# cgisky1980/Qwen3-TTS-Rust

Measured on AMD Instinct MI355X. Metric: audio_sec_per_s, higher is better.
Workload: dtype bf16

## Files before the change

include/q3tts.h:

```cpp
#ifndef Q3TTS_H
#define Q3TTS_H

#include <stdint.h>

#ifdef __cplusplus
extern "C" {
#endif

#define Q3TTS_OK 0
#define Q3TTS_ERR_INVALID (-1)
#define Q3TTS_ERR_DEVICE (-2)
#define Q3TTS_ERR_OOM (-3)
#define Q3TTS_ERR_IO (-4)
#define Q3TTS_ERR_STATE (-5)
#define Q3TTS_ERR_UNSUPPORTED (-6)
#define Q3TTS_MAX_BATCH 256

#define Q3TTS_MAX_UPSAMPLE 4
#define Q3TTS_MAX_DEC_BLOCKS 8


typedef struct q3tts_model_config {
    int32_t t_n_layer, t_d_model, t_n_head, t_n_kv_head, t_head_dim, t_d_ffn, t_vocab;
    float t_rope_theta;
// ... 334 lines not shown
int q3tts_k_bgemm_voc(int32_t device, const uint16_t* xb, int32_t B, int32_t K, const uint16_t* w_bf16, int32_t N, int32_t epilogue, const float* bias,
                      int32_t bias_n, const float* col_scale, int32_t seg_rows, int32_t gap_rows, float* y, uint16_t* yb, int32_t want_yb);
int q3tts_k_project(int32_t device, const float* x, int32_t rows, int32_t n_in, const float* w, const float* bias, int32_t n_out, const float* nw,
                    float* y, uint16_t* xb, float* ssp);
int q3tts_k_norm_inputs(int32_t device, const float* x, int32_t rows, int32_t d, const float* nw, uint16_t* xb, float* ssp);
int q3tts_k_alloc_upload(q3tts_engine* e, int64_t bytes, int64_t* mismatches);
int q3tts_k_pcm_pack(int32_t device, const float* src, int32_t rows, int64_t stride, const int32_t* ent_row, const int32_t* ent_first,
                     const int32_t* ent_count, const int64_t* ent_dst, int32_t n_ent, int32_t format, void* out, int64_t out_n);
int q3tts_k_resample_table(int32_t rate_in, int32_t rate_out, int32_t* L, int32_t* M, int32_t* H, float* tab, int64_t cap, int64_t* n);
int q3tts_k_pcm_resample(int32_t device, const float* src, int32_t rows, int64_t stride, const int32_t* row_len, const int32_t* row_final,
                         const int32_t* ent_row, const int32_t* ent_first, const int32_t* ent_count, const int64_t* ent_dst, int32_t n_ent,
                         int32_t rate_in, int32_t rate_out, int32_t format, void* out, int64_t out_n, int32_t iters, float* mean_ms);
int q3tts_k_row_buckets(int32_t max_batch, int32_t* out, int32_t cap);
int q3tts_k_bucket_steps(const q3tts_engine* e, int64_t* out, int32_t cap);
int q3tts_k_prefix_stats(const q3tts_engine* e, int64_t* out2);
int q3tts_k_engine_footprint(const q3tts_engine_config* cfg, int64_t* bytes);
int q3tts_k_device_bytes(const q3tts_engine* e, int64_t* bytes);
int q3tts_k_rng_f32(uint64_t seed, int32_t n, float* out);

#ifdef __cplusplus
}
#endif
#endif
```

qwen3-tts-rust_amd/csrc/q3_admit.hip:

```cpp
#include "q3_engine.h"

#include <chrono>
#include <cstring>

int q3_request_rules(const q3tts_request* r, bool keep, int keep_rows, const char** msg) {
    *msg = !r ? "null request"
         : keep && r->prefix ? "keep-voice: a request that names a prefix cannot keep one"
         : keep && (keep_rows < 0 || (keep_rows == 0 && (r->prompt_embd || !r->prompt))) ? "keep-voice: voice_rows >= 1 with prompt_embd (a prompt_embd request states its voice rows), >= 0 with a prompt built from ids"
         : (r->text_open == 1) && !(r->text_stream == 1) ? "text_open needs text_stream = 1"
         : (r->text_stream == 1) && (r->prompt_embd || !r->prompt || r->prompt->n_text < 1 || !r->prompt->text_ids) ? "text_stream needs a prompt built from ids (prompt), not prompt_embd, with n_text >= 1 (its first text id is the prompt's last row)"
         : "";
    return **msg ? Q3TTS_ERR_INVALID : Q3TTS_OK;
}
int q3_voice_job_rules(const q3tts_prompt_desc* p, const float* embd, int n_tok, const char** msg) {
    *msg = (p != nullptr) == (embd != nullptr) ? "give exactly one of a voice desc or host rows" : embd && n_tok < 1 ? "host rows come with n_tok >= 1" : "";
    return **msg ? Q3TTS_ERR_INVALID : Q3TTS_OK;
}
static int voice_job_check(q3tts_engine* e, const q3tts_prompt_desc* p, const float* embd, int n_tok) {
    const char* msg = "";
    if (q3_voice_job_rules(p, embd, n_tok, &msg) != Q3TTS_OK) return q3_set_err(e, Q3TTS_ERR_INVALID, std::string("prefix: ") + msg);
    if (embd && n_tok >= e->cfg.n_ctx) return q3_set_err(e, Q3TTS_ERR_INVALID, "prefix: n_tok outside 1 .. n_ctx - 1");
    return Q3TTS_OK;
}

// ... 91 lines not shown
static void copy_prefixes(q3tts_engine* e, const std::vector<Adm>& grp, Q3KvPrefix& kp) {
    int n_launch = 0; long long n_prefixed = 0;
    for (const Adm& a : grp) if (a.P > 0) { kvp_add(kp, false, a.r->prefix, a.r->prefix->P, a.b, e->stream, &n_launch); ++n_prefixed; }
    e->kvp_launches.fetch_add(n_launch + (kp.n > 0 ? 1 : 0), std::memory_order_relaxed);
    if (n_prefixed > e->kvp_group_max.load(std::memory_order_relaxed)) e->kvp_group_max.store(n_prefixed, std::memory_order_relaxed);
}
static int save_keeps(q3tts_engine* e, const std::vector<Adm>& grp, const Q3KvPrefix& kp) {
    Q3KvPrefix sv = kp; sv.n = 0;
    int bad = 0, n_launch = 0;
    for (const Adm& a : grp) if (a.keep && !bad) bad = kvp_add(sv, true, a.keep, a.keep_rows, a.b, e->stream, &n_launch);
    if (sv.n == 0) return Q3TTS_OK;
    if (bad || kvp_launch(sv, true, e->stream)) return q3_set_err(e, Q3TTS_ERR_INVALID, "prefix save: launch refused for this model shape");
    Q3_HIP(e, hipGetLastError());
    return Q3TTS_OK;
}
static int seed_slot(q3tts_engine* e, const Adm& a) {
    const q3tts_model_config& m = e->cfg.model;
    hipStream_t s = e->stream;
    const q3tts_request* r = a.r;
    const int b = a.b;
    Q3Lane& L = e->lane;
    const int row = e->row_of_slot[b];
    q3_launch_copy_rows(L.T.x + (size_t)row * m.t_d_model, m.t_d_model, e->pf.x + (size_t)(a.row0 + a.n - 1) * m.t_d_model, m.t_d_model, 1, m.t_d_model, s);
    if (q3_launch_gemm(e, e->T, q3_gemm_head(e->T, 0, m.t_vocab, e->pf, a.row0 + a.n - 1, 1, m.rms_eps, 0, L.logits + (size_t)row * m.t_vocab), s))
        return q3_set_err(e, Q3TTS_ERR_INVALID, "prefill head: launch refused for this model shape");
    float temperature = e->temperature, top_p = e->top_p; int top_k = e->top_k, has_seed = e->has_seed; uint64_t seed = e->seed;
    if (!r->use_engine_sampler) { temperature = r->temperature; top_k = r->top_k; top_p = r->top_p; has_seed = r->has_seed; seed = r->seed; }
    if (!has_seed) seed = wall_seed();
    if (temperature > 0.0f) {
        std::vector<float> draws(a.max_steps);
        q3_stdrng_f32(seed, a.max_steps, draws.data());
        Q3_HIP(e, hipMemcpyAsync(e->rng + (size_t)b * e->cfg.max_steps_cap, draws.data(), (size_t)a.max_steps * 4, hipMemcpyHostToDevice, s));
        Q3_HIP(e, hipStreamSynchronize(s));
    }
    if (e->p_temperature > 0.0f) {
        const size_t per = (size_t)(m.n_codebooks - 1), nd = (size_t)a.max_steps * per;
        std::vector<float> draws(nd);
        q3_stdrng_f32(seed ^ 0x9E3779B97F4A7C15ull, (int)nd, draws.data());
        Q3_HIP(e, hipMemcpyAsync(e->prng + (size_t)b * e->cfg.max_steps_cap * per, draws.data(), nd * 4, hipMemcpyHostToDevice, s));
        Q3_HIP(e, hipStreamSynchronize(s));
    }
    if (e->rep_penalty != 1.0f) Q3_HIP(e, hipMemsetAsync(e->seen + (size_t)b * e->seen_words, 0, (size_t)e->seen_words * 4, s));
    Q3Slot* st = e->slots_host + e->B + b;
    memset(st, 0, sizeof(*st));
    st->active = 1; st->cur_pos = a.P + a.n; st->n_frames = 0; st->max_steps = a.max_steps; st->min_frames = r->min_frames;
    st->force_eos_at = r->force_eos_at; st->top_k = top_k; st->temperature = temperature; st->top_p = top_p;
    st->rng_base = b * e->cfg.max_steps_cap;
    st->p_temperature = e->p_temperature; st->p_top_k = e->p_top_k; st->p_top_p = e->p_top_p; st->rep_penalty = e->rep_penalty;
    Q3_HIP(e, hipMemcpyAsync(e->slots + b, st, sizeof(Q3Slot), hipMemcpyHostToDevice, s));
    if (r->text_stream == 1) {
        std::vector<int32_t> T;
        q3_text_trailing(r, T);
        TRY(q3_text_rows_set(e, b, T.data(), 0, (int)T.size(), 0));
    } else if (e->ts_used) TRY(q3_text_rows_set(e, b, nullptr, 0, 0, 0));
    e->ts_slot[b] = (r->text_stream == 1) ? 1 : 0;
    if (e->voc) TRY(q3_voc_reset(e, b));
    return Q3TTS_OK;
}
static int admit_group(q3tts_engine* e, std::vector<Adm>& grp, int total) {
    if (grp.empty()) return Q3TTS_OK;
    const GroupMaps m = group_maps(grp, total);
    Q3KvPrefix kp = q3_kv_prefix_of(e->T);
    copy_prefixes(e, grp, kp);
    const int rl = prefill_layers(e, m, &kp, nullptr);
    if (rl < 0) return Q3TTS_ERR_DEVICE;
    if (rl) return q3_set_err(e, Q3TTS_ERR_INVALID, "prefill: a kernel launch was refused for this model shape");
    Q3_HIP(e, hipGetLastError());
    TRY(save_keeps(e, grp, kp));
    for (const Adm& a : grp) if (a.r) TRY(seed_slot(e, a));
    return Q3TTS_OK;
}

size_t q3_prefix_store_bytes(const q3tts_engine* e, int np) {
    const size_t per = (size_t)e->T.L * e->T.Hkv * np * e->T.hd;
    return e->T.cache.kv8 ? per + per / 16 : per * 2;
}
static Q3KvCache prefix_cache_view(const Q3Tfm& t, const q3tts_prefix* x) {
    Q3KvCache c;
    c.kc = x->k; c.vc = x->v; c.layer_stride = (size_t)t.Hkv * x->np * t.hd; c.n_ctx = x->np; c.n_slots = 1; c.kv8 = t.cache.kv8;
    if (c.kv8) { const size_t quants = t.L * c.layer_stride; c.kd = (uint16_t*)((int8_t*)x->k + quants); c.vd = (uint16_t*)((int8_t*)x->v + quants); }
    return c;
}
static int prefix_store_alloc(q3tts_engine* e, q3tts_prefix* x, int rows) {
    if (e->T.hd != Q3_ATT_HD) return q3_set_err(e, Q3TTS_ERR_INVALID, "prefix: the save kernel needs head_dim 128");
// ... 131 lines not shown
```

qwen3-tts-rust_amd/csrc/q3_engine.h:

```cpp
#pragma once
#include <algorithm>
#include <cstddef>
#include <atomic>
#include <mutex>
#include <string>
#include <vector>

#include "../../include/q3tts.h"
#include "q3_kernels.h"

static_assert(sizeof(q3tts_request) == 80 && offsetof(q3tts_request, text_stream) == 12 && offsetof(q3tts_request, prompt) == 16 &&
              offsetof(q3tts_request, text_open) == 44 && offsetof(q3tts_request, seed) == 48 && offsetof(q3tts_request, prefix) == 72, "q3tts_request layout");

struct Q3Voc;
struct Q3Mel;
struct Q3Clone;

struct Q3KvCache {
    uint16_t *kc = nullptr, *vc = nullptr;
    size_t layer_stride = 0;
    bool kv8 = false; uint16_t *kd = nullptr, *vd = nullptr;
    int n_ctx = 0, n_slots = 0;
};

// ... 59 lines not shown
    float* tts_pad = nullptr;
    float* marker_row = nullptr;
    int B = 0;
    std::vector<int> buckets; int cur_bucket = -1;
    std::vector<std::atomic<long long>> bucket_steps;
    std::atomic<long long> kvp_launches{0}, kvp_group_max{0};
    std::vector<int> row_of_slot, slot_of_row;
    Q3Slot* slots = nullptr;
    Q3Slot* slots_host = nullptr;
    int* codes = nullptr;
    float* rng = nullptr;
    Q3Lane lane;
    Q3Scratch sc_pre;
    Q3Rows pf;
    int *pf_pos = nullptr, *pf_slot = nullptr;
    int* pf_seg = nullptr;
    Q3PromptRow* prow_dev = nullptr; int prow_cap = 0;
    float* spk_dev = nullptr; int* refcodes_dev = nullptr;
    float temperature = 0.7f; int top_k = 40; float top_p = 0.9f; int has_seed = 0; uint64_t seed = 0;
    int max_steps = 512;
    float p_temperature = 0.0f; int p_top_k = 0; float p_top_p = 1.0f; float rep_penalty = 1.0f;
    int pred_force = 0, pred_variant = 0;
    int streams_open = 0;
    int* ts_ids = nullptr; int* ts_cnt = nullptr; int2* ts_cur = nullptr;
    std::vector<char> ts_slot; int ts_variant = 0, ts_used = 0;
    float* prng = nullptr;
    uint32_t* seen = nullptr; int seen_words = 0;
    hipEvent_t ev0 = nullptr, ev1 = nullptr, ev2 = nullptr, ev3 = nullptr;
    std::vector<hipEvent_t> fin_ev;
    q3tts_timings tm{};
// ... 87 lines not shown
int q3_capture_frames(q3tts_engine* e, std::vector<hipGraph_t>& graphs, std::vector<hipGraphExec_t>& execs);
Q3BGemm q3_gemm_qkv(const Q3Tfm& t, int l, const Q3Rows& r, const Q3Scratch& sc, int rows, float eps, int once);
Q3BGemm q3_gemm_head(const Q3Tfm& t, int q, int N, const Q3Rows& r, int row0, int rows, float eps, int once, float* y);
int q3_launch_gemm(q3tts_engine* e, const Q3Tfm& t, const Q3BGemm& g, hipStream_t s, hipEvent_t* probe = nullptr, int kind = -1);

void q3_rope_tables(int n_pos, int hd, float theta, const int* sections, std::vector<float>& cs, std::vector<float>& sn);

void q3_stdrng_f32(uint64_t seed, int n, float* out);

void q3_mel_destroy(q3tts_engine* e);
int q3_mel_run(q3tts_engine* e, const float* audio, int64_t n_samples, int32_t* n_frames, float** out_dev);
void q3_clone_destroy(q3tts_engine* e);
int q3_voc_create(q3tts_engine* e);
void q3_voc_destroy(q3tts_engine* e);
int q3_voc_reset(q3tts_engine* e, int slot);
int q3_voc_decode(q3tts_engine* e, int slot, int f0, int nf, int is_last, hipStream_t s);
int q3_voc_decode_batch(q3tts_engine* e, const int* slots, const int* real, int ns, int nf, hipStream_t s, int beside_decoder);
void q3_voc_mark_last(q3tts_engine* e, int slot);
float* q3_voc_pcm(q3tts_engine* e, int slot);
int q3_voc_samples(q3tts_engine* e, int slot);
int q3_voc_samples_per_frame(const q3tts_engine* e);
size_t q3_voc_pcm_stride(const q3tts_engine* e);
struct Q3SlotBlock { char* base; unsigned long long stride, bytes; };
void q3_voc_slot_blocks(q3tts_engine* e, std::vector<Q3SlotBlock>& out);
void q3_voc_host_state(q3tts_engine* e, int slot, int* frames_done, int* last_flag, bool set);

struct Q3Swap;
int q3_swap_create(q3tts_engine* e, long long arena_bytes, Q3Swap** out);
void q3_swap_destroy(q3tts_engine* e, Q3Swap* sw);
long long q3_swap_block_bytes(const q3tts_engine* e, const Q3Swap* sw, int cur_pos, int voc_frames);
// ... 13 lines not shown

enum { PROMPT_WHOLE = 0, PROMPT_VOICE = 1, PROMPT_TEXT = 2 };
int build_prompt_dev(q3tts_engine* e, const q3tts_prompt_desc* p, float* out, int max_rows, int* n_out, int part = PROMPT_WHOLE, bool text_stream = false);

int q3_plan_rows(q3tts_engine* e, const std::vector<int>& live);
int q3_admit_many(q3tts_engine* e, const int* slots, const q3tts_request* const* reqs, int count, int* rc);
int q3_admit(q3tts_engine* e, int b, const q3tts_request* r);
int q3_request_rules(const q3tts_request* r, bool keep, int keep_rows, const char** msg);
int q3_voice_job_rules(const q3tts_prompt_desc* p, const float* embd, int n_tok, const char** msg);
struct Q3AdmItem {
    int slot; const q3tts_request* r;
    q3tts_prefix* keep; int keep_rows;
    const q3tts_prompt_desc* voice; const float* embd; int n_tok;
};
int q3_admit_items(q3tts_engine* e, const Q3AdmItem* items, int count, int* rc);
int q3_run_chunk(q3tts_engine* e, int CH, float* dev_ms = nullptr);
int q3_codes_back(q3tts_engine* e, int b, q3tts_result* o);
int q3_retire_slot(q3tts_engine* e, int b, hipStream_t evs);
int q3_emit_count(const q3tts_engine* e, int ns, bool done, long long delivered);
void q3_prefix_free(q3tts_prefix* x);
int q3_clone_audio_encode_run(q3tts_engine* e, const float* audio, int64_t n_samples, int64_t* codes, int32_t cap_frames, int32_t* n_frames);
int q3_clone_speaker_encode_run(q3tts_engine* e, const float* audio, int64_t n_samples, float* spk_emb);
int q3_resample_run(q3tts_engine* e, const float* in, int64_t n_in, int32_t rate_in, int32_t rate_out, float* out, int64_t cap, int64_t* n_out);
int q3_text_rows_set(q3tts_engine* e, int b, const int32_t* T, int from, int n, int n_frames);
int q3_park_rows(q3tts_engine* e, int b, bool save);
void q3_text_trailing(const q3tts_request* r, std::vector<int32_t>& T);
int q3_pred_force_variant(q3tts_engine* e, int force);
int q3_voc_dispatch(q3tts_engine* e, const char* live, const char* want, int* voc_frames, bool more, bool* first);
double q3_now_ms();
```

qwen3-tts-rust_amd/csrc/q3_engine.hip:

```cpp
#include "q3_engine.h"
#include "q3_gguf.h"

#include <chrono>
#include <cmath>
#include <cstdio>
#include <cstdlib>
#include <cstring>

static thread_local std::string g_err;

int q3_set_err(q3tts_engine* e, int code, const std::string& msg) {
    if (e) { std::lock_guard<std::mutex> lk(e->err_mu); e->err = msg; }
    g_err = msg;
    return code;
}
extern "C" const char* q3tts_last_error(const q3tts_engine* e) {
    if (!e) return g_err.c_str();
    if (!e->session.load()) return e->err.c_str();
    static thread_local std::string copy;
    std::lock_guard<std::mutex> lk(const_cast<q3tts_engine*>(e)->err_mu);
    copy = e->err;
    return copy.c_str();
}
int q3_refuse_in_session(q3tts_engine* e) {
// ... 122 lines not shown
    if (err != hipSuccess) { hipFree(q); return q3_set_err(e, Q3TTS_ERR_DEVICE, std::string("hipMemset: ") + hipGetErrorString(err)); }
    if (e) e->dev_bytes += bytes;
    *p = q;
    return Q3TTS_OK;
}
extern "C" int q3tts_k_bucket_steps(const q3tts_engine* e, int64_t* out, int32_t cap) {
    if (!e || !out || cap < (int)e->bucket_steps.size()) return q3_set_err(nullptr, Q3TTS_ERR_INVALID, "bucket steps: null argument or output too small");
    for (size_t i = 0; i < e->bucket_steps.size(); ++i) out[i] = e->bucket_steps[i].load(std::memory_order_relaxed);
    return (int)e->bucket_steps.size();
}
extern "C" int q3tts_k_prefix_stats(const q3tts_engine* e, int64_t* out2) {
    if (!e || !out2) return q3_set_err(nullptr, Q3TTS_ERR_INVALID, "null argument");
    out2[0] = e->kvp_launches.load(std::memory_order_relaxed); out2[1] = e->kvp_group_max.load(std::memory_order_relaxed);
    return Q3TTS_OK;
}
extern "C" int q3tts_k_device_bytes(const q3tts_engine* e, int64_t* bytes) {
    if (!e || !bytes) return q3_set_err(nullptr, Q3TTS_ERR_INVALID, "null argument");
    *bytes = (int64_t)e->dev_bytes;
    return Q3TTS_OK;
}
static int alloc_scratch(q3tts_engine* e, Q3Scratch& sc, int rows, int nqkv, int nq, int F) {
    sc.rows = rows;
    const size_t r16 = ((size_t)rows + 15) & ~(size_t)15;
    TRY(q3_dalloc(e, &sc.qkv, (size_t)rows * nqkv)); TRY(q3_dalloc(e, &sc.att, r16 * nq)); TRY(q3_dalloc(e, &sc.h, r16 * F));
    sc.rt16 = (int)(r16 / 16);
    if (e->T.a8 || e->P.a8) { TRY(q3_dalloc(e, &sc.asc_att, r16 * (nq / 32))); TRY(q3_dalloc(e, &sc.asc_h, r16 * (F / 32))); }
    return Q3TTS_OK;
}

static int alloc_rows(q3tts_engine* e, Q3Rows& r, size_t rows, int d, bool scales) {
// ... 59 lines not shown
    e->B = B;
    hipStream_t s = e->stream;
    const std::string wdir = cfg->weights_path ? cfg->weights_path : "";
    Q3Gguf gt, gp;
    std::string er;
    if (!wdir.empty() && (gt.open(wdir + "/qwen3_tts_talker.gguf", er) || gp.open(wdir + "/qwen3_tts_predictor.gguf", er))) { q3_set_err(e, Q3TTS_ERR_INVALID, er); return fail(Q3TTS_ERR_INVALID); }
    TRYC(q3_tfm_init(e, e->T, {.grp = Q3G_TALKER, .L = m.t_n_layer, .d = m.t_d_model, .Hq = m.t_n_head, .Hkv = m.t_n_kv_head, .hd = m.t_head_dim, .F = m.t_d_ffn,
                               .head_n = m.t_vocab, .theta = m.t_rope_theta, .sections = m.t_mrope_sections, .n_ctx = cfg->n_ctx, .n_slots = B, .kv8 = cfg->kv_q8_0},
                     wdir.empty() ? nullptr : &gt, "qwen3_tts_talker.gguf", cfg->talker_q8_0));
    TRYC(q3_tfm_init(e, e->P, {.grp = Q3G_PRED, .L = m.p_n_layer, .d = m.p_d_model, .Hq = m.p_n_head, .Hkv = m.p_n_kv_head, .hd = m.p_head_dim, .F = m.p_d_ffn,
                               .head_n = (m.n_codebooks - 1) * m.codebook_size, .theta = m.p_rope_theta, .sections = nullptr, .n_ctx = 64, .n_slots = B, .kv8 = 0},
                     wdir.empty() ? nullptr : &gp, "qwen3_tts_predictor.gguf", cfg->predictor_q8_0));
    TRYC(q3_assets_init(e, wdir));
    TRYC(q3_pred_table_init(e));
    TRYC(q3_dalloc(e, &e->slots, (size_t)B));
    HIPC(hipHostMalloc((void**)&e->slots_host, sizeof(Q3Slot) * 2 * B, hipHostMallocDefault));
    memset(e->slots_host, 0, sizeof(Q3Slot) * 2 * B);
    TRYC(q3_dalloc(e, &e->codes, (size_t)B * cfg->max_steps_cap * m.n_codebooks)); TRYC(q3_dalloc(e, &e->rng, (size_t)B * cfg->max_steps_cap));
    TRYC(q3_dalloc(e, &e->prng, (size_t)B * cfg->max_steps_cap * (m.n_codebooks - 1)));
    e->seen_words = (m.sample_limit + 31) / 32;
    TRYC(q3_dalloc(e, &e->seen, (size_t)B * e->seen_words));
    TRYC(q3_dalloc(e, &e->ts_ids, (size_t)B * cfg->max_steps_cap)); TRYC(q3_dalloc(e, &e->ts_cnt, (size_t)B)); TRYC(q3_dalloc(e, &e->ts_cur, (size_t)B));
    TRYC(q3_dalloc(e, &e->park_logits, (size_t)B * m.t_vocab)); TRYC(q3_dalloc(e, &e->park_x, (size_t)B * m.t_d_model));
    e->ts_slot.assign(B, 0);
    {
        const int nb = B;
        const int nqkv_max = std::max(e->T.nqkv, e->P.nqkv), nq_max = std::max(e->T.nq, e->P.nq), F_max = std::max(e->T.F, e->P.F);
        Q3Lane& L = e->lane;
        L.nb = nb;
        HIPC(hipStreamCreateWithFlags(&L.stream, hipStreamNonBlocking));
        HIPC(hipEventCreate(&L.ev_begin)); HIPC(hipEventCreate(&L.ev_end));
// ... 4 lines not shown
        TRYC(q3_dalloc(e, &L.row_pos_t, (size_t)nb)); TRYC(q3_dalloc(e, &L.slot_id, (size_t)nb)); TRYC(q3_dalloc(e, &L.perm, (size_t)nb));
        std::vector<int> sid(nb), rp(nb, -1);
        for (int b = 0; b < nb; ++b) sid[b] = b;
        HIPC(hipMemcpyAsync(L.slot_id, sid.data(), nb * 4, hipMemcpyHostToDevice, s));
        HIPC(hipMemcpyAsync(L.row_pos_t, rp.data(), nb * 4, hipMemcpyHostToDevice, s));
        HIPC(hipStreamSynchronize(s));
        TRYC(alloc_scratch(e, L.sc, 2 * nb, nqkv_max, nq_max, F_max));
        row_buckets(nb, e->buckets);
        e->bucket_steps = std::vector<std::atomic<long long>>(e->buckets.size());
        e->cur_bucket = (int)e->buckets.size() - 1;
        e->row_of_slot = sid; e->slot_of_row = sid;
    }
    TRYC(alloc_scratch(e, e->sc_pre, cfg->n_ctx, e->T.nqkv, e->T.nq, e->T.F));
    TRYC(alloc_rows(e, e->pf, (size_t)cfg->n_ctx, m.t_d_model, e->T.a8));
    TRYC(q3_dalloc(e, &e->pf_pos, (size_t)cfg->n_ctx)); TRYC(q3_dalloc(e, &e->pf_slot, (size_t)cfg->n_ctx)); TRYC(q3_dalloc(e, &e->pf_seg, (size_t)4 * cfg->max_batch));
    { std::vector<int> pp(cfg->n_ctx); for (int i = 0; i < cfg->n_ctx; ++i) pp[i] = i;
      HIPC(hipMemcpyAsync(e->pf_pos, pp.data(), pp.size() * 4, hipMemcpyHostToDevice, s)); HIPC(hipStreamSynchronize(s)); }
    e->prow_cap = cfg->n_ctx;
    TRYC(q3_dalloc(e, &e->prow_dev, (size_t)e->prow_cap)); TRYC(q3_dalloc(e, &e->spk_dev, (size_t)m.d_embed));
    TRYC(q3_dalloc(e, &e->refcodes_dev, (size_t)cfg->n_ctx * 16));
    {
        TRYC(q3_dalloc(e, &e->marker_row, (size_t)m.d_embed));
        const Q3PromptRow mr{1, m.tts_pad_id, 0, 0};
        HIPC(hipMemcpyAsync(e->prow_dev, &mr, sizeof(mr), hipMemcpyHostToDevice, s));
        HIPC(hipStreamSynchronize(s));
        q3_launch_prompt_rows(e->prow_dev, 1, e->text, m.text_vocab, e->codec_dev, m.codec0_rows, m.codecq_rows, m.n_codebooks, e->spk_dev, m.d_embed, e->marker_row, s);
        HIPC(hipStreamSynchronize(s));
    }
    if (cfg->with_vocoder) {
        TRYC(q3_voc_create(e));
// ... 23 lines not shown
        for (auto ge : L.execs) if (ge) hipGraphExecDestroy(ge);
        for (auto gr : L.graphs) if (gr) hipGraphDestroy(gr);
        for (auto ge : L.execs_s) if (ge) hipGraphExecDestroy(ge);
        for (auto gr : L.graphs_s) if (gr) hipGraphDestroy(gr);
        for (int v = 0; v < 2; ++v) {
            for (auto ge : L.execs_t[v]) if (ge) hipGraphExecDestroy(ge);
            for (auto gr : L.graphs_t[v]) if (gr) hipGraphDestroy(gr);
        }
        if (L.ev_begin) hipEventDestroy(L.ev_begin); if (L.ev_end) hipEventDestroy(L.ev_end);
        if (L.stream) hipStreamDestroy(L.stream);
    }
    for (void* p : e->allocs) hipFree(p);
    hipFree(e->dev_pcm);
    hipFree(e->rs_stage);
    if (e->slots_host) hipHostFree(e->slots_host);
    for (auto ev : e->fin_ev) if (ev) hipEventDestroy(ev);
    for (auto ev : e->probe_ev) if (ev) hipEventDestroy(ev);
    if (e->ev0) hipEventDestroy(e->ev0); if (e->ev1) hipEventDestroy(e->ev1); if (e->ev2) hipEventDestroy(e->ev2); if (e->ev3) hipEventDestroy(e->ev3);
    if (e->stream) hipStreamDestroy(e->stream);
    if (e->vstream && e->vstream != e->stream) hipStreamDestroy(e->vstream);
    delete e;
}

extern "C" int q3tts_set_sampler(q3tts_engine* e, float temperature, int32_t top_k, float top_p, int32_t has_seed, uint64_t seed) {
    if (!e) return q3_set_err(nullptr, Q3TTS_ERR_INVALID, "null engine");
    Q3_NOT_IN_SESSION(e);
    e->temperature = temperature; e->top_k = top_k; e->top_p = top_p; e->has_seed = has_seed; e->seed = seed;
    return Q3TTS_OK;
}
static int refuse_busy(q3tts_engine* e) {
// ... 164 lines not shown
```

qwen3-tts-rust_amd/csrc/q3_vocoder.hip:

```cpp
#include <algorithm>
#include <cmath>
#include <map>
#include <set>
#include <tuple>
#include <vector>

#include "q3_engine.h"

typedef __bf16 bf16x8 __attribute__((ext_vector_type(8)));

#define VOC_MAX_NS 64
#define VOC_FCAP 4

enum { VC_CODEBOOK = 0, VC_PRE = 32, VC_TFM = 40, VC_FINAL_NORM = 60, VC_UP = 64, VC_DEC_IN = 72, VC_BLK = 80, VC_OUT = 120 };
enum { VW_W = 0, VW_B = 1, VW_IN_NORM = 2, VW_Q = 3, VW_K = 4, VW_V = 5, VW_O = 6, VW_LS_ATTN = 7, VW_POST_NORM = 8, VW_GATE = 9,
       VW_UP = 10, VW_DOWN = 11, VW_LS_MLP = 12, VW_DW_W = 13, VW_DW_B = 14, VW_LN_W = 15, VW_LN_B = 16, VW_PW1 = 17, VW_PW1_B = 18,
       VW_PW2 = 19, VW_PW2_B = 20, VW_GAMMA = 21, VW_ALPHA = 22, VW_BETA = 23, VW_W2 = 24, VW_B2 = 25, VW_ALPHA2 = 26, VW_BETA2 = 27 };
#define VTID(l, w) Q3_TID(Q3G_VOC, l, w)

struct VCall {
    int ns, nf;
    int slot[VOC_MAX_NS];
    int pos[VOC_MAX_NS];
};
// ... 1349 lines not shown
    return tab;
}
void q3_voc_slot_blocks(q3tts_engine* e, std::vector<Q3SlotBlock>& out) {
    const Q3Voc* v = e->voc;
    out = voc_hist_blocks(v);
    const unsigned long long ring = (unsigned long long)v->RW * v->c.n_head * v->c.head_dim * 4;
    for (int l = 0; l < v->c.n_layer; ++l)
        for (float* r : {v->kring, v->vring}) out.push_back({(char*)r + (unsigned long long)l * v->B * ring, ring, ring});
}
void q3_voc_host_state(q3tts_engine* e, int slot, int* frames_done, int* last_flag, bool set) {
    Q3Voc* v = e->voc;
    if (set) { v->frames_done[slot] = *frames_done; v->last_flag[slot] = *last_flag; }
    else { *frames_done = v->frames_done[slot]; *last_flag = v->last_flag[slot]; }
}

__global__ void k_voc_zero(const Q3Voc::ZeroEnt* tab, int slot) {
    const Q3Voc::ZeroEnt z = tab[blockIdx.x];
    uint32_t* p = (uint32_t*)(z.base + (size_t)slot * z.bytes);
    const size_t n = z.bytes / 4;
    for (size_t i = (size_t)blockIdx.y * blockDim.x + threadIdx.x; i < n; i += (size_t)gridDim.y * blockDim.x) p[i] = 0u;
}
int q3_voc_reset(q3tts_engine* e, int slot) {
    Q3Voc* v = e->voc;
    if (!v) return Q3TTS_OK;
    if (!v->zero_tab) {
        std::vector<Q3Voc::ZeroEnt> tab;
        for (const Q3SlotBlock& h : voc_hist_blocks(v)) tab.push_back({h.base, h.bytes});
        v->n_zero = (int)tab.size();
        VTRY(valloc(e, v, &v->zero_tab, tab.size()));
        Q3_HIP(e, hipMemcpy(v->zero_tab, tab.data(), tab.size() * sizeof(Q3Voc::ZeroEnt), hipMemcpyHostToDevice));
    }
    if (v->n_zero) hipLaunchKernelGGL(k_voc_zero, dim3(v->n_zero, 4), dim3(256), 0, e->stream, v->zero_tab, slot);
    v->frames_done[slot] = 0; v->last_flag[slot] = 0;
    return Q3TTS_OK;
}

struct VSnake { VRows to; const float* ea = nullptr; const float* ib = nullptr; int n = 1; };
static VSnake snake_into(const VBuf& dst, const float* ea, const float* ib, int C) { return {dst.rows(), ea, ib, C}; }
struct VOpt {
    const float* scale = nullptr; int scale_n = 1;
    VSnake snake;
    int store = 1;
    VOpt& layer_scale(const float* v, int n) { scale = v; scale_n = n; return *this; }
    VOpt& snake_to(const VSnake& k) { snake = k; return *this; }
    VOpt& no_store() { store = 0; return *this; }
};
static bool vconv_chunked(const VConv& c) { return c.ntap == 7 && c.cin % 64 == 0 && c.cin >= 256; }
static bool voc_ring_ok(const VLaunch& vl, const VGemm& g) { return !vl.no_ring && g.c.nout % 4 == 0 && g.y_off % 4 == 0 && g.y_stride % 4 == 0 && g.y2_off % 4 == 0 && g.y2_stride % 4 == 0; }
// ... 442 lines not shown
```

qwen3-tts-rust_amd/q3tts/_abi.py:

```python
import ctypes as C
import os

HERE = os.path.dirname(os.path.abspath(__file__))
PKG_ROOT = os.path.dirname(HERE)
REPO_ROOT = os.path.dirname(PKG_ROOT)
LIB_PATH = os.path.join(PKG_ROOT, "csrc", "libq3tts.so")

Q3TTS_MAX_UPSAMPLE = 4
Q3TTS_MAX_DEC_BLOCKS = 8


class ModelConfig(C.Structure):
    _fields_ = [
        ("t_n_layer", C.c_int32), ("t_d_model", C.c_int32), ("t_n_head", C.c_int32), ("t_n_kv_head", C.c_int32),
        ("t_head_dim", C.c_int32), ("t_d_ffn", C.c_int32), ("t_vocab", C.c_int32),
        ("t_rope_theta", C.c_float),
        ("t_mrope_sections", C.c_int32 * 4),
        ("p_n_layer", C.c_int32), ("p_d_model", C.c_int32), ("p_n_head", C.c_int32), ("p_n_kv_head", C.c_int32),
        ("p_head_dim", C.c_int32), ("p_d_ffn", C.c_int32),
        ("p_rope_theta", C.c_float),
        ("n_codebooks", C.c_int32), ("codebook_size", C.c_int32),
        ("rms_eps", C.c_float),
        ("d_embed", C.c_int32), ("text_vocab", C.c_int32), ("codec0_rows", C.c_int32), ("codecq_rows", C.c_int32),
        ("sample_limit", C.c_int32), ("eos_code", C.c_int32), ("tts_pad_id", C.c_int32),
# ... 135 lines not shown
    "q3tts_session_last_error", "q3tts_k_pcm_pack",
    "q3tts_prefix_create", "q3tts_prefix_rows", "q3tts_prefix_destroy", "q3tts_k_talker_prefill_prefix",
    "q3tts_config_from_model_dir", "q3tts_k_gguf_meta",
    "q3tts_set_predictor_sampler", "q3tts_get_predictor_sampler", "q3tts_set_repetition_penalty", "q3tts_get_repetition_penalty",
    "q3tts_k_pred_variant",
    "q3tts_set_output_rate", "q3tts_get_output_rate", "q3tts_resample", "q3tts_k_resample_table", "q3tts_k_pcm_resample",
    "q3tts_session_append_text", "q3tts_k_text_ready",
    "q3tts_k_attention_runs", "q3tts_k_attention_decode_ex", "q3tts_k_attention_pair", "q3tts_k_attend_pick",
    "q3tts_k_attention_runs_kv8", "q3tts_k_attention_decode_kv8", "q3tts_k_attend_pick_kv8",
    "q3tts_k_pred_table_row", "q3tts_k_pred_next", "q3tts_k_attention_gather",
    "q3tts_k_row_buckets", "q3tts_k_bucket_steps", "q3tts_k_device_bytes", "q3tts_k_engine_footprint", "q3tts_k_prefix_stats",
    "q3tts_session_prefix_create", "q3tts_session_submit_keep_voice", "q3tts_session_prefix_release", "q3tts_session_clone",
    "q3tts_prefix_state", "q3tts_k_prefix_read",
    "q3tts_session_submit_paced", "q3tts_session_grant", "q3tts_session_set_swap", "q3tts_session_swap_stats",
    "q3tts_k_credit_ready", "q3tts_k_swap_arena", "q3tts_k_swap_phase_ms",
    "q3tts_k_request_rules",
]


class PredStep(C.Structure):
    _fields_ = [
        ("n_rows", C.c_int32), ("q", C.c_int32), ("n_codebooks", C.c_int32), ("n_key_parts", C.c_int32), ("rows_q", C.c_int32),
        ("d_embed", C.c_int32), ("d_proj", C.c_int32), ("max_steps_cap", C.c_int32),
        ("keys", C.c_void_p), ("active", C.c_void_p), ("n_frames", C.c_void_p), ("codec_q", C.c_void_p), ("pproj_q", C.c_void_p),
        ("proj_b", C.c_void_p), ("fb", C.c_void_p), ("px", C.c_void_p), ("codes", C.c_void_p),
    ]


class Q3Error(RuntimeError):
    pass

# ... 146 lines not shown
    lib.q3tts_node_shard.restype = C.c_int32
    lib.q3tts_k_bgemm_q8.argtypes = [C.c_int32, C.c_void_p, C.c_int32, C.c_int32, C.c_void_p, C.c_void_p, C.c_int32, C.c_void_p, C.c_int32, C.c_int32, C.c_float,
                                     C.c_int32, C.c_void_p, C.c_void_p, C.c_void_p, C.c_void_p, C.c_void_p, C.c_int32, f32p]
    lib.q3tts_k_bgemm_q8a8_argmax.argtypes = [C.c_int32, C.c_void_p, C.c_void_p, C.c_int32, C.c_int32, C.c_void_p, C.c_void_p, C.c_int32, C.c_void_p, C.c_int32, C.c_int32, C.c_float, C.c_void_p]
    lib.q3tts_k_bgemm_q8a8_argmax.restype = C.c_int
    lib.q3tts_k_bgemm_q8a8.argtypes = [C.c_int32, C.c_void_p, C.c_void_p, C.c_int32, C.c_int32, C.c_void_p, C.c_void_p, C.c_int32, C.c_void_p, C.c_int32, C.c_int32, C.c_float,
                                       C.c_int32, C.c_void_p, C.c_void_p, C.c_void_p, C.c_void_p, C.c_void_p, C.c_int32, f32p]
    lib.q3tts_k_bgemm_policy.argtypes = [C.c_int32]
    lib.q3tts_k_attend_policy.argtypes = [C.c_int32, C.c_int32]
    lib.q3tts_k_bgemm_pick.argtypes = [C.c_int32, C.c_int32, C.c_int32, C.c_int32, C.c_int32, C.c_int32, i32p]
    lib.q3tts_k_alloc_upload.argtypes = [vp, C.c_int64, C.POINTER(C.c_int64)]
    lib.q3tts_k_row_buckets.argtypes = [C.c_int32, i32p, C.c_int32]
    lib.q3tts_k_bucket_steps.argtypes = [vp, C.POINTER(C.c_int64), C.c_int32]
    lib.q3tts_k_device_bytes.argtypes = [vp, C.POINTER(C.c_int64)]
    lib.q3tts_k_prefix_stats.argtypes = [vp, C.POINTER(C.c_int64)]
    lib.q3tts_k_engine_footprint.argtypes = [C.POINTER(EngineConfig), C.POINTER(C.c_int64)]
    lib.q3tts_tokenizer_load.argtypes = [C.c_char_p, C.POINTER(vp), C.c_char_p, C.c_int32]
    lib.q3tts_tokenizer_free.argtypes = [vp]
    lib.q3tts_tokenizer_free.restype = None
    lib.q3tts_tokenizer_vocab_size.argtypes = [vp]
    lib.q3tts_tokenizer_vocab_size.restype = C.c_int32
    lib.q3tts_tokenizer_encode.argtypes = [vp, C.c_char_p, C.c_int64, u32p, C.c_int32, i32p, C.c_char_p, C.c_int32]
    lib.q3tts_tokenizer_decode.argtypes = [vp, u32p, C.c_int32, C.c_char_p, C.c_int64, C.POINTER(C.c_int64), C.c_char_p, C.c_int32]
    if path is None:
        _lib = lib
    return lib


def default_config():
    cfg = EngineConfig()
# ... 105 lines not shown
```

qwen3-tts-rust_amd/q3tts/native.py:

```python
import ctypes as C
import math
import os
import weakref

import numpy as np

from . import _abi

f32p, i32p, u32p = C.POINTER(C.c_float), C.POINTER(C.c_int32), C.POINTER(C.c_uint32)


def _ptr(a, typ):
    return a.ctypes.data_as(typ)


_LANG_DEFAULT = object()


def make_prompt_desc(text_ids, spk_emb=None, lang_id=_LANG_DEFAULT, spk_id=-1, instruct_ids=None, ref_codes=None,
                     ref_text_ids=None, part="whole"):
    if part not in ("whole", "voice", "text"):
        raise ValueError(f"part must be 'whole', 'voice' or 'text', not {part!r}")
    if part == "voice" and text_ids is not None and len(text_ids) > 0:
        raise ValueError("a voice-only desc has no text: text_ids must be None or empty")
# ... 209 lines not shown
    def row_buckets(self):
        return row_buckets(self.cfg.max_batch)

    def bucket_steps(self):
        out = (C.c_int64 * 32)()
        n = self.lib.q3tts_k_bucket_steps(self.h, out, 32)
        if n < 0:
            raise _abi.Q3Error("q3tts_k_bucket_steps failed")
        return dict(zip(self.row_buckets(), [int(out[i]) for i in range(n)]))

    def prefix_stats(self):
        o = (C.c_int64 * 2)()
        self._check(self.lib.q3tts_k_prefix_stats(self.h, o), "q3tts_k_prefix_stats")
        return int(o[0]), int(o[1])

    def device_bytes(self):
        b = C.c_int64(0)
        self._check(self.lib.q3tts_k_device_bytes(self.h, C.byref(b)), "q3tts_k_device_bytes")
        return int(b.value)

    def timings(self):
        t = _abi.Timings()
        self._check(self.lib.q3tts_get_timings(self.h, C.byref(t)), "q3tts_get_timings")
        return t

    def mel(self, audio):
        a = np.ascontiguousarray(audio, dtype=np.float32)
        cap = int(self.lib.q3tts_mel_frames(a.size))
        out = np.zeros((max(cap, 1), 128), dtype=np.float32)
        n = C.c_int32(0)
# ... 954 lines not shown
```

Before: 694.4.

## Batch per-slot admission seeding into grouped kernels with pinned staging

```diff
diff --git a/include/q3tts.h b/include/q3tts.h
--- a/include/q3tts.h
+++ b/include/q3tts.h
@@ -372,6 +372,7 @@
 int q3tts_k_row_buckets(int32_t max_batch, int32_t* out, int32_t cap);
 int q3tts_k_bucket_steps(const q3tts_engine* e, int64_t* out, int32_t cap);
 int q3tts_k_prefix_stats(const q3tts_engine* e, int64_t* out2);
+int q3tts_k_admit_stats(const q3tts_engine* e, int64_t* out4);
 int q3tts_k_engine_footprint(const q3tts_engine_config* cfg, int64_t* bytes);
 int q3tts_k_device_bytes(const q3tts_engine* e, int64_t* bytes);
 int q3tts_k_rng_f32(uint64_t seed, int32_t n, float* out);
diff --git a/qwen3-tts-rust_amd/csrc/q3_admit.hip b/qwen3-tts-rust_amd/csrc/q3_admit.hip
--- a/qwen3-tts-rust_amd/csrc/q3_admit.hip
+++ b/qwen3-tts-rust_amd/csrc/q3_admit.hip
@@ -129,6 +129,118 @@
     Q3_HIP(e, hipGetLastError());
     return Q3TTS_OK;
 }
+struct AdmSampler { float temperature, top_p; int top_k; uint64_t seed; };
+static AdmSampler adm_sampler(const q3tts_engine* e, const q3tts_request* r) {
+    AdmSampler sm{e->temperature, e->top_p, e->top_k, e->seed};
+    int has_seed = e->has_seed;
+    if (!r->use_engine_sampler) { sm.temperature = r->temperature; sm.top_k = r->top_k; sm.top_p = r->top_p; has_seed = r->has_seed; sm.seed = r->seed; }
+    if (!has_seed) sm.seed = wall_seed();
+    return sm;
+}
+static Q3Slot* slot_record(q3tts_engine* e, const Adm& a, const AdmSampler& sm) {
+    const int b = a.b;
+    Q3Slot* st = e->slots_host + e->B + b;
+    memset(st, 0, sizeof(*st));
+    st->active = 1; st->cur_pos = a.P + a.n; st->n_frames = 0; st->max_steps = a.max_steps; st->min_frames = a.r->min_frames;
+    st->force_eos_at = a.r->force_eos_at; st->top_k = sm.top_k; st->temperature = sm.temperature; st->top_p = sm.top_p;
+    st->rng_base = b * e->cfg.max_steps_cap;
+    st->p_temperature = e->p_temperature; st->p_top_k = e->p_top_k; st->p_top_p = e->p_top_p; st->rep_penalty = e->rep_penalty;
+    return st;
+}
+
+struct Q3AdmEnt { int src_row, lane_row, slot, n_draws, n_pdraws, pad[3]; };
+static_assert(sizeof(Q3AdmEnt) == 32 && sizeof(Q3Slot) % 4 == 0, "staging layout");
+struct AdmStage { Q3AdmEnt* ent; int* slots; float* draws; float* pdraws; size_t bytes; };
+static AdmStage adm_stage(const q3tts_engine* e, char* base) {
+    const size_t B = (size_t)e->cfg.max_batch, cap = (size_t)e->cfg.max_steps_cap, per = (size_t)(e->cfg.model.n_codebooks - 1);
+    AdmStage st;
+    st.ent = (Q3AdmEnt*)base; st.slots = (int*)(st.ent + B);
+    st.draws = (float*)(base + ((B * (sizeof(Q3AdmEnt) + 4) + 255) & ~(size_t)255)); st.pdraws = st.draws + B * cap;
+    st.bytes = (size_t)((char*)(st.pdraws + B * cap * per) - base);
+    return st;
+}
+size_t q3_adm_stage_bytes(const q3tts_engine* e) { return adm_stage(e, nullptr).bytes; }
+
+struct Q3AdmGather { const Q3AdmEnt* ent; const float* x; const uint16_t* xb; const float* ssp; float* lane_x; uint16_t* cxb; float* cssp; int d; };
+__global__ __launch_bounds__(256) void k_admit_gather(Q3AdmGather a) {
+    const int i = blockIdx.x, d = a.d, kb = d >> 5, nt = d >> 4;
+    const Q3AdmEnt en = a.ent[i];
+    for (int k = threadIdx.x; k < d; k += 256) {
+        a.lane_x[(size_t)en.lane_row * d + k] = a.x[(size_t)en.src_row * d + k];
+        a.cxb[q3_atile_off(i, k, kb)] = a.xb[q3_atile_off(en.src_row, k, kb)];
+    }
+    for (int t = threadIdx.x; t < nt; t += 256) a.cssp[(size_t)i * nt + t] = a.ssp[(size_t)en.src_row * nt + t];
+}
+struct Q3AdmTail {
+    const Q3AdmEnt* ent; const float* clogits; float* logits; int vocab;
+    const float* draws; float* rng; int cap; const float* pdraws; float* prng; int pcap;
+    uint32_t* seen; int seen_words; const Q3Slot* recs; Q3Slot* slots;
+};
+__global__ __launch_bounds__(256) void k_admit_tail(Q3AdmTail a) {
+    const int i = blockIdx.x, t0 = blockIdx.y * 256 + threadIdx.x, step = gridDim.y * 256;
+    const Q3AdmEnt en = a.ent[i];
+    for (int k = t0; k < a.vocab; k += step) a.logits[(size_t)en.lane_row * a.vocab + k] = a.clogits[(size_t)i * a.vocab + k];
+    for (int k = t0; k < en.n_draws; k += step) a.rng[(size_t)en.slot * a.cap + k] = a.draws[(size_t)i * a.cap + k];
+    for (int k = t0; k < en.n_pdraws; k += step) a.prng[(size_t)en.slot * a.pcap + k] = a.pdraws[(size_t)i * a.pcap + k];
+    if (a.seen) for (int k = t0; k < a.seen_words; k += step) a.seen[(size_t)en.slot * a.seen_words + k] = 0u;
+    if (blockIdx.y == 0)
+        for (int k = threadIdx.x; k < (int)(sizeof(Q3Slot) / 4); k += 256) ((uint32_t*)(a.slots + en.slot))[k] = ((const uint32_t*)(a.recs + en.slot))[k];
+}
+static int seed_group(q3tts_engine* e, const std::vector<Adm>& grp) {
+    const q3tts_model_config& m = e->cfg.model;
+    hipStream_t s = e->stream;
+    Q3Lane& L = e->lane;
+    int n = 0;
+    for (const Adm& a : grp) if (a.r) ++n;
+    if (n == 0) return Q3TTS_OK;
+    long long launches = 0, syncs = 0;
+    if (e->adm_busy) {
+        if (hipEventQuery(e->adm_ev) != hipSuccess) { (void)hipGetLastError(); Q3_HIP(e, hipEventSynchronize(e->adm_ev)); ++syncs; }
+        e->adm_busy = false;
+    }
+    const AdmStage h = adm_stage(e, e->adm_host), dv = adm_stage(e, e->adm_dev);
+    const size_t cap = (size_t)e->cfg.max_steps_cap, per = (size_t)(m.n_codebooks - 1);
+    std::vector<Q3TextSet> texts; std::vector<std::vector<int32_t>> trailing(n);
+    int i = 0;
+    for (const Adm& a : grp) {
+        if (!a.r) continue;
+        const AdmSampler sm = adm_sampler(e, a.r);
+        Q3AdmEnt& en = h.ent[i];
+        en = Q3AdmEnt{a.row0 + a.n - 1, e->row_of_slot[a.b], a.b, 0, 0, {0, 0, 0}};
+        h.slots[i] = a.b;
+        if (sm.temperature > 0.0f) { en.n_draws = a.max_steps; q3_stdrng_f32(sm.seed, a.max_steps, h.draws + (size_t)i * cap); }
+        if (e->p_temperature > 0.0f) {
+            en.n_pdraws = (int)((size_t)a.max_steps * per);
+            q3_stdrng_f32(sm.seed ^ 0x9E3779B97F4A7C15ull, en.n_pdraws, h.pdraws + (size_t)i * cap * per);
+        }
+        slot_record(e, a, sm);
+        if (a.r->text_stream == 1) { q3_text_trailing(a.r, trailing[i]); texts.push_back(Q3TextSet{a.b, trailing[i].data(), 0, (int)trailing[i].size(), 0}); }
+        else if (e->ts_used) texts.push_back(Q3TextSet{a.b, nullptr, 0, 0, 0});
+        e->ts_slot[a.b] = (a.r->text_stream == 1) ? 1 : 0;
+        ++i;
+    }
+    const int d = m.t_d_model;
+    hipLaunchKernelGGL(k_admit_gather, dim3(n), dim3(256), 0, s, Q3AdmGather{dv.ent, e->pf.x, e->pf.xb, e->pf.ssp, L.T.x, e->adm.xb, e->adm.ssp, d});
+    if (q3_launch_gemm(e, e->T, q3_gemm_head(e->T, 0, m.t_vocab, e->adm, 0, n, m.rms_eps, 0, e->adm_logits), s))
+        return q3_set_err(e, Q3TTS_ERR_INVALID, "prefill head: launch refused for this model shape");
+    Q3AdmTail t{dv.ent, e->adm_logits, L.logits, m.t_vocab, dv.draws, e->rng, (int)cap, dv.pdraws, e->prng, (int)(cap * per),
+                e->rep_penalty != 1.0f ? e->seen : nullptr, e->seen_words, e->slots_stage_dev, e->slots};
+    hipLaunchKernelGGL(k_admit_tail, dim3(n, 4), dim3(256), 0, s, t);
+    launches += 3;
+    if (e->voc) { TRY(q3_voc_reset_group(e, h.slots, dv.slots, n)); ++launches; }
+    Q3_HIP(e, hipGetLastError());
+    Q3_HIP(e, hipEventRecord(e->adm_ev, s));
+    e->adm_busy = true;
+    if (!texts.empty()) {
+        TRY(q3_text_rows_set_group(e, texts.data(), (int)texts.size()));
+        for (const Q3TextSet& it : texts) launches += it.T ? 3 : 2;
+        ++syncs;
+    }
+    e->adm_stats[0].fetch_add(launches, std::memory_order_relaxed); e->adm_stats[1].fetch_add(syncs, std::memory_order_relaxed);
+    e->adm_stats[2].fetch_add(1, std::memory_order_relaxed);
+    return Q3TTS_OK;
+}
+
 static int seed_slot(q3tts_engine* e, const Adm& a) {
     const q3tts_model_config& m = e->cfg.model;
     hipStream_t s = e->stream;
@@ -139,30 +251,28 @@
     q3_launch_copy_rows(L.T.x + (size_t)row * m.t_d_model, m.t_d_model, e->pf.x + (size_t)(a.row0 + a.n - 1) * m.t_d_model, m.t_d_model, 1, m.t_d_model, s);
     if (q3_launch_gemm(e, e->T, q3_gemm_head(e->T, 0, m.t_vocab, e->pf, a.row0 + a.n - 1, 1, m.rms_eps, 0, L.logits + (size_t)row * m.t_vocab), s))
         return q3_set_err(e, Q3TTS_ERR_INVALID, "prefill head: launch refused for this model shape");
-    float temperature = e->temperature, top_p = e->top_p; int top_k = e->top_k, has_seed = e->has_seed; uint64_t seed = e->seed;
-    if (!r->use_engine_sampler) { temperature = r->temperature; top_k = r->top_k; top_p = r->top_p; has_seed = r->has_seed; seed = r->seed; }
-    if (!has_seed) seed = wall_seed();
-    if (temperature > 0.0f) {
+    const AdmSampler sm = adm_sampler(e, r);
+    long long launches = 2, syncs = 0;
+    if (sm.temperature > 0.0f) {
         std::vector<float> draws(a.max_steps);
-        q3_stdrng_f32(seed, a.max_steps, draws.data());
+        q3_stdrng_f32(sm.seed, a.max_steps, draws.data());
         Q3_HIP(e, hipMemcpyAsync(e->rng + (size_t)b * e->cfg.max_steps_cap, draws.data(), (size_t)a.max_steps * 4, hipMemcpyHostToDevice, s));
         Q3_HIP(e, hipStreamSynchronize(s));
+        ++launches; ++syncs;
     }
     if (e->p_temperature > 0.0f) {
         const size_t per = (size_t)(m.n_codebooks - 1), nd = (size_t)a.max_steps * per;
         std::vector<float> draws(nd);
-        q3_stdrng_f32(seed ^ 0x9E3779B97F4A7C15ull, (int)nd, draws.data());
+        q3_stdrng_f32(sm.seed ^ 0x9E3779B97F4A7C15ull, (int)nd, draws.data());
         Q3_HIP(e, hipMemcpyAsync(e->prng + (size_t)b * e->cfg.max_steps_cap * per, draws.data(), nd * 4, hipMemcpyHostToDevice, s));
         Q3_HIP(e, hipStreamSynchronize(s));
-    }
-    if (e->rep_penalty != 1.0f) Q3_HIP(e, hipMemsetAsync(e->seen + (size_t)b * e->seen_words, 0, (size_t)e->seen_words * 4, s));
-    Q3Slot* st = e->slots_host + e->B + b;
-    memset(st, 0, sizeof(*st));
-    st->active = 1; st->cur_pos = a.P + a.n; st->n_frames = 0; st->max_steps = a.max_steps; st->min_frames = r->min_frames;
-    st->force_eos_at = r->force_eos_at; st->top_k = top_k; st->temperature = temperature; st->top_p = top_p;
-    st->rng_base = b * e->cfg.max_steps_cap;
-    st->p_temperature = e->p_temperature; st->p_top_k = e->p_top_k; st->p_top_p = e->p_top_p; st->rep_penalty = e->rep_penalty;
-    Q3_HIP(e, hipMemcpyAsync(e->slots + b, st, sizeof(Q3Slot), hipMemcpyHostToDevice, s));
+        ++launches; ++syncs;
+    }
+    if (e->rep_penalty != 1.0f) { Q3_HIP(e, hipMemsetAsync(e->seen + (size_t)b * e->seen_words, 0, (size_t)e->seen_words * 4, s)); ++launches; }
+    Q3_HIP(e, hipMemcpyAsync(e->slots + b, slot_record(e, a, sm), sizeof(Q3Slot), hipMemcpyHostToDevice, s));
+    launches += 1 + (e->voc ? 1 : 0);
+    if (r->text_stream == 1 || e->ts_used) { launches += r->text_stream == 1 ? 3 : 2; ++syncs; }
+    e->adm_stats[0].fetch_add(launches, std::memory_order_relaxed); e->adm_stats[1].fetch_add(syncs, std::memory_order_relaxed);
     if (r->text_stream == 1) {
         std::vector<int32_t> T;
         q3_text_trailing(r, T);
@@ -182,7 +292,10 @@
     if (rl) return q3_set_err(e, Q3TTS_ERR_INVALID, "prefill: a kernel launch was refused for this model shape");
     Q3_HIP(e, hipGetLastError());
     TRY(save_keeps(e, grp, kp));
-    for (const Adm& a : grp) if (a.r) TRY(seed_slot(e, a));
+    if (e->admit_batched && !e->T.a8) return seed_group(e, grp);
+    bool any = false;
+    for (const Adm& a : grp) if (a.r) { TRY(seed_slot(e, a)); any = true; }
+    if (any) e->adm_stats[3].fetch_add(1, std::memory_order_relaxed);
     return Q3TTS_OK;
 }
 
diff --git a/qwen3-tts-rust_amd/csrc/q3_engine.h b/qwen3-tts-rust_amd/csrc/q3_engine.h
--- a/qwen3-tts-rust_amd/csrc/q3_engine.h
+++ b/qwen3-tts-rust_amd/csrc/q3_engine.h
@@ -97,6 +97,11 @@
     Q3Scratch sc_pre;
     Q3Rows pf;
     int *pf_pos = nullptr, *pf_slot = nullptr;
+    int admit_batched = 1;
+    Q3Rows adm; float* adm_logits = nullptr;
+    char *adm_host = nullptr, *adm_dev = nullptr; Q3Slot* slots_stage_dev = nullptr;
+    hipEvent_t adm_ev = nullptr; bool adm_busy = false;
+    std::atomic<long long> adm_stats[4] = {};
     int* pf_seg = nullptr;
     Q3PromptRow* prow_dev = nullptr; int prow_cap = 0;
     float* spk_dev = nullptr; int* refcodes_dev = nullptr;
@@ -214,6 +219,7 @@
 int q3_voc_create(q3tts_engine* e);
 void q3_voc_destroy(q3tts_engine* e);
 int q3_voc_reset(q3tts_engine* e, int slot);
+int q3_voc_reset_group(q3tts_engine* e, const int* slots, const int* slots_dev, int n);
 int q3_voc_decode(q3tts_engine* e, int slot, int f0, int nf, int is_last, hipStream_t s);
 int q3_voc_decode_batch(q3tts_engine* e, const int* slots, const int* real, int ns, int nf, hipStream_t s, int beside_decoder);
 void q3_voc_mark_last(q3tts_engine* e, int slot);
@@ -257,6 +263,7 @@
     const q3tts_prompt_desc* voice; const float* embd; int n_tok;
 };
 int q3_admit_items(q3tts_engine* e, const Q3AdmItem* items, int count, int* rc);
+size_t q3_adm_stage_bytes(const q3tts_engine* e);
 int q3_run_chunk(q3tts_engine* e, int CH, float* dev_ms = nullptr);
 int q3_codes_back(q3tts_engine* e, int b, q3tts_result* o);
 int q3_retire_slot(q3tts_engine* e, int b, hipStream_t evs);
diff --git a/qwen3-tts-rust_amd/csrc/q3_engine.hip b/qwen3-tts-rust_amd/csrc/q3_engine.hip
--- a/qwen3-tts-rust_amd/csrc/q3_engine.hip
+++ b/qwen3-tts-rust_amd/csrc/q3_engine.hip
@@ -160,6 +160,11 @@
     out2[0] = e->kvp_launches.load(std::memory_order_relaxed); out2[1] = e->kvp_group_max.load(std::memory_order_relaxed);
     return Q3TTS_OK;
 }
+extern "C" int q3tts_k_admit_stats(const q3tts_engine* e, int64_t* out4) {
+    if (!e || !out4) return q3_set_err(nullptr, Q3TTS_ERR_INVALID, "null argument");
+    for (int i = 0; i < 4; ++i) out4[i] = e->adm_stats[i].load(std::memory_order_relaxed);
+    return Q3TTS_OK;
+}
 extern "C" int q3tts_k_device_bytes(const q3tts_engine* e, int64_t* bytes) {
     if (!e || !bytes) return q3_set_err(nullptr, Q3TTS_ERR_INVALID, "null argument");
     *bytes = (int64_t)e->dev_bytes;
@@ -249,7 +254,7 @@
     TRYC(q3_assets_init(e, wdir));
     TRYC(q3_pred_table_init(e));
     TRYC(q3_dalloc(e, &e->slots, (size_t)B));
-    HIPC(hipHostMalloc((void**)&e->slots_host, sizeof(Q3Slot) * 2 * B, hipHostMallocDefault));
+    HIPC(hipHostMalloc((void**)&e->slots_host, sizeof(Q3Slot) * 2 * B, hipHostMallocMapped));
     memset(e->slots_host, 0, sizeof(Q3Slot) * 2 * B);
     TRYC(q3_dalloc(e, &e->codes, (size_t)B * cfg->max_steps_cap * m.n_codebooks)); TRYC(q3_dalloc(e, &e->rng, (size_t)B * cfg->max_steps_cap));
     TRYC(q3_dalloc(e, &e->prng, (size_t)B * cfg->max_steps_cap * (m.n_codebooks - 1)));
@@ -284,6 +289,15 @@
     TRYC(alloc_scratch(e, e->sc_pre, cfg->n_ctx, e->T.nqkv, e->T.nq, e->T.F));
     TRYC(alloc_rows(e, e->pf, (size_t)cfg->n_ctx, m.t_d_model, e->T.a8));
     TRYC(q3_dalloc(e, &e->pf_pos, (size_t)cfg->n_ctx)); TRYC(q3_dalloc(e, &e->pf_slot, (size_t)cfg->n_ctx)); TRYC(q3_dalloc(e, &e->pf_seg, (size_t)4 * cfg->max_batch));
+    {
+        const char* ev = getenv("Q3TTS_ADMIT_BATCHED");
+        e->admit_batched = (ev && !atoi(ev)) ? 0 : 1;
+        TRYC(alloc_rows(e, e->adm, (size_t)B, m.t_d_model, false)); TRYC(q3_dalloc(e, &e->adm_logits, (size_t)B * m.t_vocab));
+        HIPC(hipHostMalloc((void**)&e->adm_host, q3_adm_stage_bytes(e), hipHostMallocMapped));
+        HIPC(hipHostGetDevicePointer((void**)&e->adm_dev, e->adm_host, 0));
+        HIPC(hipHostGetDevicePointer((void**)&e->slots_stage_dev, e->slots_host + B, 0));
+        HIPC(hipEventCreateWithFlags(&e->adm_ev, hipEventDisableTiming));
+    }
     { std::vector<int> pp(cfg->n_ctx); for (int i = 0; i < cfg->n_ctx; ++i) pp[i] = i;
       HIPC(hipMemcpyAsync(e->pf_pos, pp.data(), pp.size() * 4, hipMemcpyHostToDevice, s)); HIPC(hipStreamSynchronize(s)); }
     e->prow_cap = cfg->n_ctx;
@@ -337,6 +351,8 @@
     hipFree(e->dev_pcm);
     hipFree(e->rs_stage);
     if (e->slots_host) hipHostFree(e->slots_host);
+    if (e->adm_host) hipHostFree(e->adm_host);
+    if (e->adm_ev) hipEventDestroy(e->adm_ev);
     for (auto ev : e->fin_ev) if (ev) hipEventDestroy(ev);
     for (auto ev : e->probe_ev) if (ev) hipEventDestroy(ev);
     if (e->ev0) hipEventDestroy(e->ev0); if (e->ev1) hipEventDestroy(e->ev1); if (e->ev2) hipEventDestroy(e->ev2); if (e->ev3) hipEventDestroy(e->ev3);
diff --git a/qwen3-tts-rust_amd/csrc/q3_vocoder.hip b/qwen3-tts-rust_amd/csrc/q3_vocoder.hip
--- a/qwen3-tts-rust_amd/csrc/q3_vocoder.hip
+++ b/qwen3-tts-rust_amd/csrc/q3_vocoder.hip
@@ -1387,24 +1387,36 @@
     else { *frames_done = v->frames_done[slot]; *last_flag = v->last_flag[slot]; }
 }
 
-__global__ void k_voc_zero(const Q3Voc::ZeroEnt* tab, int slot) {
+__global__ void k_voc_zero(const Q3Voc::ZeroEnt* tab, const int* slots, int slot) {
     const Q3Voc::ZeroEnt z = tab[blockIdx.x];
+    if (slots) slot = slots[blockIdx.z];
     uint32_t* p = (uint32_t*)(z.base + (size_t)slot * z.bytes);
     const size_t n = z.bytes / 4;
     for (size_t i = (size_t)blockIdx.y * blockDim.x + threadIdx.x; i < n; i += (size_t)gridDim.y * blockDim.x) p[i] = 0u;
 }
+static int voc_zero_tab(q3tts_engine* e, Q3Voc* v) {
+    if (v->zero_tab) return Q3TTS_OK;
+    std::vector<Q3Voc::ZeroEnt> tab;
+    for (const Q3SlotBlock& h : voc_hist_blocks(v)) tab.push_back({h.base, h.bytes});
+    v->n_zero = (int)tab.size();
+    VTRY(valloc(e, v, &v->zero_tab, tab.size()));
+    Q3_HIP(e, hipMemcpy(v->zero_tab, tab.data(), tab.size() * sizeof(Q3Voc::ZeroEnt), hipMemcpyHostToDevice));
+    return Q3TTS_OK;
+}
 int q3_voc_reset(q3tts_engine* e, int slot) {
     Q3Voc* v = e->voc;
     if (!v) return Q3TTS_OK;
-    if (!v->zero_tab) {
-        std::vector<Q3Voc::ZeroEnt> tab;
-        for (const Q3SlotBlock& h : voc_hist_blocks(v)) tab.push_back({h.base, h.bytes});
-        v->n_zero = (int)tab.size();
-        VTRY(valloc(e, v, &v->zero_tab, tab.size()));
-        Q3_HIP(e, hipMemcpy(v->zero_tab, tab.data(), tab.size() * sizeof(Q3Voc::ZeroEnt), hipMemcpyHostToDevice));
-    }
-    if (v->n_zero) hipLaunchKernelGGL(k_voc_zero, dim3(v->n_zero, 4), dim3(256), 0, e->stream, v->zero_tab, slot);
+    VTRY(voc_zero_tab(e, v));
+    if (v->n_zero) hipLaunchKernelGGL(k_voc_zero, dim3(v->n_zero, 4), dim3(256), 0, e->stream, v->zero_tab, (const int*)nullptr, slot);
     v->frames_done[slot] = 0; v->last_flag[slot] = 0;
+    return Q3TTS_OK;
+}
+int q3_voc_reset_group(q3tts_engine* e, const int* slots, const int* slots_dev, int n) {
+    Q3Voc* v = e->voc;
+    if (!v || n <= 0) return Q3TTS_OK;
+    VTRY(voc_zero_tab(e, v));
+    if (v->n_zero) hipLaunchKernelGGL(k_voc_zero, dim3(v->n_zero, 4, n), dim3(256), 0, e->stream, v->zero_tab, slots_dev, 0);
+    for (int i = 0; i < n; ++i) { v->frames_done[slots[i]] = 0; v->last_flag[slots[i]] = 0; }
     return Q3TTS_OK;
 }
 
diff --git a/qwen3-tts-rust_amd/q3tts/_abi.py b/qwen3-tts-rust_amd/q3tts/_abi.py
--- a/qwen3-tts-rust_amd/q3tts/_abi.py
+++ b/qwen3-tts-rust_amd/q3tts/_abi.py
@@ -173,7 +173,7 @@
     "q3tts_prefix_state", "q3tts_k_prefix_read",
     "q3tts_session_submit_paced", "q3tts_session_grant", "q3tts_session_set_swap", "q3tts_session_swap_stats",
     "q3tts_k_credit_ready", "q3tts_k_swap_arena", "q3tts_k_swap_phase_ms",
-    "q3tts_k_request_rules",
+    "q3tts_k_request_rules", "q3tts_k_admit_stats",
 ]
 
 
@@ -350,6 +350,7 @@
     lib.q3tts_k_bucket_steps.argtypes = [vp, C.POINTER(C.c_int64), C.c_int32]
     lib.q3tts_k_device_bytes.argtypes = [vp, C.POINTER(C.c_int64)]
     lib.q3tts_k_prefix_stats.argtypes = [vp, C.POINTER(C.c_int64)]
+    lib.q3tts_k_admit_stats.argtypes = [vp, C.POINTER(C.c_int64)]
     lib.q3tts_k_engine_footprint.argtypes = [C.POINTER(EngineConfig), C.POINTER(C.c_int64)]
     lib.q3tts_tokenizer_load.argtypes = [C.c_char_p, C.POINTER(vp), C.c_char_p, C.c_int32]
     lib.q3tts_tokenizer_free.argtypes = [vp]
diff --git a/qwen3-tts-rust_amd/q3tts/native.py b/qwen3-tts-rust_amd/q3tts/native.py
--- a/qwen3-tts-rust_amd/q3tts/native.py
+++ b/qwen3-tts-rust_amd/q3tts/native.py
@@ -247,6 +247,11 @@
         self._check(self.lib.q3tts_k_prefix_stats(self.h, o), "q3tts_k_prefix_stats")
         return int(o[0]), int(o[1])
 
+    def admit_stats(self):
+        o = (C.c_int64 * 4)()
+        self._check(self.lib.q3tts_k_admit_stats(self.h, o), "q3tts_k_admit_stats")
+        return dict(zip(("launches", "syncs", "batched", "per_slot"), (int(x) for x in o)))
+
     def device_bytes(self):
         b = C.c_int64(0)
         self._check(self.lib.q3tts_k_device_bytes(self.h, C.byref(b)), "q3tts_k_device_bytes")
```

Measured after the change: 684.1. 0.985x the previous value.
